# isxml/YOLO-SOMI

Measured on AMD Instinct MI355X. Metric: images/sec train (forward+loss+backward+Adam+EMA) @640, VisDrone-shaped synthetic, yolov5l-SOMI (DCNv3 blocks), higher is better.
Workload: dtype f32; 1 GPU; yolov5l-SOMI (DCNv3 blocks) training step: uint8 ingest + forward (batch-stat BN) + ComputeLoss + backward + Adam + EMA, 640x640, batch 32/GPU (BASELINE configs[1] shape); batch_per_gpu=32, imgsz=640, params=77918970, classes=10, parallelism=dp1

## Files before the change

### yolo-somi_amd/csrc/common.h

```cpp
#pragma once
#include <hip/hip_runtime.h>
#include <stdint.h>
#include <stdio.h>
#include <initializer_list>
#include "../../include/somi_hip.h"

namespace somi {

void set_error(const char *fmt, ...);

#define SOMI_REQUIRE(cond, code, ...)            \
    do {                                         \
        if (!(cond)) {                           \
            ::somi::set_error(__VA_ARGS__);      \
            return (code);                       \
        }                                        \
    } while (0)

static inline int launch_status(const char *what) {
    hipError_t e = hipGetLastError();
    if (e != hipSuccess) {
        set_error("%s: launch failed: %s", what, hipGetErrorString(e));
        return (int)e;
    }
    return 0;
}

static inline bool aligned16(const void *p) { return (reinterpret_cast<uintptr_t>(p) & 15u) == 0; }
static inline int cdiv(long a, long b) { return (int)((a + b - 1) / b); }
static inline int r4(int c) { return (c + 3) / 4 * 4; }
static inline size_t align_up(size_t v, size_t a) { return (v + a - 1) / a * a; }

static inline const char *slice_fault(const void *p, int cs, int coff, int width) {
    if (!p) return "null pointer";
    if (!aligned16(p)) return "base not 16-byte aligned";
    if (cs <= 0 || cs % 4) return "channel stride not a positive multiple of 4";
    if (coff < 0 || coff % 4) return "channel offset not a non-negative multiple of 4";
    if (width <= 0) return "no channels";
    if ((long)coff + width > cs) return "runs past the channel stride";
    return nullptr;
}

struct Slice { const char *name; const void *p; int cs, coff, width; bool optional; };
constexpr bool kOptional = true;
static inline int slices_status(const char *who, std::initializer_list<Slice> slices) {
    for (const Slice &s : slices)
        if (const char *why = s.optional && !s.p ? nullptr : slice_fault(s.p, s.cs, s.coff, s.width)) {
            set_error("%s: %s = [%d, %ld) of %d channels: %s", who, s.name, s.coff, (long)s.coff + s.width, s.cs, why);
            return SOMI_EINVAL;
        }
    return 0;
}
#define SOMI_REQUIRE_SLICES(who, ...)                                          \
    do {                                                                       \
        if (::somi::slices_status(who, {__VA_ARGS__})) return SOMI_EINVAL;     \
    } while (0)

constexpr int kNumXCD = 8;

void launch_dwconv3x3(bool flip, const float *x, const float *w, const float *bias, const float *ps, const float *pt, const float *res,
                      float *y, int B, int H, int W, int C, int act, hipStream_t s);

__device__ __forceinline__ int xcd_remap(int bid, int nblk) {
    const int q = nblk / kNumXCD, r = nblk % kNumXCD;
    const int xcd = bid % kNumXCD, idx = bid / kNumXCD;
    const int start = xcd < r ? xcd * (q + 1) : r * (q + 1) + (xcd - r) * q;
    return start + idx;
}

__device__ __forceinline__ float sigmoidf_(float v) { return 1.0f / (1.0f + expf(-v)); }

__device__ __forceinline__ void bifpn_norm(const float *__restrict__ w, int n_in, float eps, float (&wn)[3]) {
    float s = 0.f;
    for (int i = 0; i < n_in; ++i) s += w[i] * (1.0f / (1.0f + expf(-w[i])));
    for (int i = 0; i < 3; ++i) wn[i] = i < n_in ? w[i] / (s + eps) : 0.f;
}

template <int ACT>
__device__ __forceinline__ float apply_act(float v) {
    if constexpr (ACT == SOMI_ACT_SILU) return v / (1.0f + expf(-v));
    else if constexpr (ACT == SOMI_ACT_GELU) return 0.5f * v * (1.0f + erff(v * 0.70710678118654752440f));
    else if constexpr (ACT == SOMI_ACT_RELU) return fmaxf(v, 0.0f);
    else if constexpr (ACT == SOMI_ACT_SIGMOID) return 1.0f / (1.0f + expf(-v));
    else if constexpr (ACT == SOMI_ACT_LEAKY) return v > 0.0f ? v : 0.1f * v;
    else return v;
}

__device__ __forceinline__ float apply_act_rt(float v, int act) {
    switch (act) {
        case SOMI_ACT_SILU: return apply_act<SOMI_ACT_SILU>(v);
        case SOMI_ACT_GELU: return apply_act<SOMI_ACT_GELU>(v);
        case SOMI_ACT_RELU: return apply_act<SOMI_ACT_RELU>(v);
        case SOMI_ACT_SIGMOID: return apply_act<SOMI_ACT_SIGMOID>(v);
        case SOMI_ACT_LEAKY: return apply_act<SOMI_ACT_LEAKY>(v);
        default: return v;
    }
}

}
```

### yolo-somi_amd/csrc/conv_igemm.hip

```cpp
#include "common.h"

namespace somi {

typedef float f32x16 __attribute__((ext_vector_type(16)));
typedef float f32x4 __attribute__((ext_vector_type(4)));
typedef unsigned u32x4 __attribute__((ext_vector_type(4)));
typedef unsigned u32x2 __attribute__((ext_vector_type(2)));
typedef __bf16 bf16x8 __attribute__((ext_vector_type(8)));

constexpr int BK = 32;
constexpr int OP_LD = BK;
constexpr unsigned OOB = 0xFFFFFFE0u;
constexpr unsigned OOB_BASE = 0xF0000000u;
constexpr unsigned MAX_BUF_BYTES = 0xE0000000u;

__device__ __forceinline__ void lds_dma16(__amdgpu_buffer_rsrc_t r, float *lds_base, unsigned voff) {
#if defined(__HIP_DEVICE_COMPILE__)
    __builtin_amdgcn_raw_ptr_buffer_load_lds(r, (__attribute__((address_space(3))) void *)lds_base, 16, voff, 0, 0, 0);
#endif
}
__device__ __forceinline__ void lds_dma_wait() {
#if defined(__HIP_DEVICE_COMPILE__)
    asm volatile("s_waitcnt vmcnt(0)" ::: "memory");
#endif
// ... 201 lines not shown
        for (int i = 0; i < A_ROWS; ++i) a_par[i] = 0;
#pragma unroll
        for (int i = 0; i < A_ROWS; ++i) {
            const int m = m0 + row0 + RPP * i;
            if (m < Mrows) {
                const int b = m / HoWo + bz, rem = m % HoWo;
                const int ho = h0 + (rem / Wc) * cstep, wo = w0 + (rem % Wc) * cstep;
                if (!a.dgrad) {
                    a_hi0[i] = ho * d.stride - d.pad;
                    a_wi0[i] = wo * d.stride - d.pad;
                } else {
                    a_hi0[i] = (ho + d.pad) / d.stride;
                    a_wi0[i] = (wo + d.pad) / d.stride;
                    a_par[i] = ((ho + d.pad) % d.stride) | (((wo + d.pad) % d.stride) << 8);
                }
                a_pixi[i] = (b * d.H + a_hi0[i]) * d.W + a_wi0[i];
                a_off[i] = a_pixi[i] * d.x_cs + d.x_coff;
                a_chn[i] = b * d.Cin;
            } else {
                a_hi0[i] = -(1 << 28);
                a_wi0[i] = 0; a_pixi[i] = 0; a_off[i] = 0; a_chn[i] = 0;
            }
        }
        unsigned b_off[B_ROWS];
#pragma unroll
        for (int i = 0; i < B_ROWS; ++i) {
            const int n = n0 + row0 + RPP * i;
            b_off[i] = n < d.Cout ? (unsigned)(((size_t)bz * d.Cout + n) * a.K + kc) * 4u : (FAST ? OOB_BASE : OOB);
        }
        unsigned a_mask[A_ROWS], a_offb[A_ROWS], a_pixb[A_ROWS], a_chnb[A_ROWS];
        if constexpr (FAST) {
            const int ntap = nr_c * nq_c;
#pragma unroll
            for (int i = 0; i < A_ROWS; ++i) {
                unsigned mk = 0;
                for (int t = 0; t < ntap; ++t) {
                    const int tr = t / nq_c, tq = t % nq_c;
                    const int hh = a_hi0[i] + (cls ? -tr : tr * d.dil);
                    const int ww = a_wi0[i] + (cls ? -tq : tq * d.dil);
                    mk |= ((unsigned)hh < (unsigned)d.H && (unsigned)ww < (unsigned)d.W) ? (1u << t) : 0u;
                }
                a_mask[i] = mk;
                a_offb[i] = (unsigned)(a_off[i] + kc) * 4u;
                a_pixb[i] = (unsigned)a_pixi[i] * 4u;
                a_chnb[i] = (unsigned)(a_chn[i] + kc) * 4u;
            }
        }
        const int ntap_u = FAST ? nr_c * nq_c : 1;
        int tp_u = FAST ? kt0 % ntap_u : 0, c0_u = FAST ? (kt0 / ntap_u) * BK : 0;
        int r_u = tp_u / nq_c, q_u = tp_u % nq_c;

        int k = kc, c = kc % d.Cin, tap = kc / d.Cin;
        int r = tap / d.kw, q = tap % d.kw;

        f32x4 ra[A_ROWS], rb[B_ROWS];
        auto fetch_tile = [&](int kt_next) {
            if constexpr (FAST) {
                const int dpix = cls ? -(r_u * d.W + q_u) : (r_u * d.W + q_u) * d.dil;
                const unsigned sd = (unsigned)(dpix * d.x_cs + c0_u) * 4u, bit = 1u << tp_u;
#pragma unroll
                for (int i = 0; i < A_ROWS; ++i) {
                    const bool ok = (a_mask[i] & bit) != 0;
                    f32x4 v = buf_load4(rx, ok ? a_offb[i] + sd : OOB);
                    if constexpr (MODULATE) {
                        if (has_chan) v *= buf_load4(rc, ok ? a_chnb[i] + (unsigned)c0_u * 4u : OOB);
                        if (has_pix) v *= buf_load1(rp, ok ? a_pixb[i] + (unsigned)dpix * 4u : OOB);
                    }
                    ra[i] = v;
                }
                const unsigned ko = cls ? (unsigned)(((ph + cstep * r_u) * d.kw + pw + cstep * q_u) * d.Cin + c0_u) * 4u
                                        : (unsigned)(tp_u * d.Cin + c0_u) * 4u;
#pragma unroll
                for (int i = 0; i < B_ROWS; ++i) rb[i] = buf_load4(rw, b_off[i] + ko);
                return;
            }
            const bool kin = k < a.K;
            const int dh = a.dgrad ? -(r / d.stride) : r * d.dil, dw = a.dgrad ? -(q / d.stride) : q * d.dil;
            const int dpix = dh * d.W + dw;
            const int delta = dpix * d.x_cs + c;
            const int rpar = a.dgrad ? ((r % d.stride) | ((q % d.stride) << 8)) : 0;
#pragma unroll
            for (int i = 0; i < A_ROWS; ++i) {
                const bool ok = kin && a_par[i] == rpar && (unsigned)(a_hi0[i] + dh) < (unsigned)d.H &&
                                (unsigned)(a_wi0[i] + dw) < (unsigned)d.W;
                f32x4 v = buf_load4(rx, ok ? (unsigned)(a_off[i] + delta) * 4u : OOB);
                if constexpr (MODULATE) {
                    if (has_chan) v *= buf_load4(rc, ok ? (unsigned)(a_chn[i] + c) * 4u : OOB);
                    if (has_pix) v *= buf_load1(rp, ok ? (unsigned)(a_pixi[i] + dpix) * 4u : OOB);
                }
                ra[i] = v;
            }
#pragma unroll
            for (int i = 0; i < B_ROWS; ++i) rb[i] = buf_load4(rw, (kin && b_off[i] != OOB) ? b_off[i] : OOB);
        };
        auto advance_k = [&]() {
            if constexpr (FAST) {
                ++tp_u;
                if (++q_u == nq_c) { q_u = 0; ++r_u; }
                if (tp_u == ntap_u) {
                    tp_u = 0; r_u = 0; q_u = 0;
                    c0_u += BK;
                }
                return;
            }
            k += BK;
            c += BK;
            while (c >= d.Cin) {
                c -= d.Cin;
                if (++q == d.kw) { q = 0; ++r; }
            }
#pragma unroll
            for (int i = 0; i < B_ROWS; ++i) b_off[i] += (b_off[i] != OOB) ? BK * 4u : 0u;
        };
        auto store_split = [&](float *rowp, const f32x4 &v) {
            const __bf16 h0 = (__bf16)v[0], h1 = (__bf16)v[1], h2 = (__bf16)v[2], h3 = (__bf16)v[3];
            typedef __bf16 bf16x4 __attribute__((ext_vector_type(4)));
            *reinterpret_cast<bf16x4 *>(rowp + st_off) = bf16x4{h0, h1, h2, h3};
            if constexpr (NS == 2) {
                const bf16x4 lo = {(__bf16)(v[0] - (float)h0), (__bf16)(v[1] - (float)h1), (__bf16)(v[2] - (float)h2), (__bf16)(v[3] - (float)h3)};
                *reinterpret_cast<bf16x4 *>(rowp + (st_off ^ 16)) = lo;
            }
        };
        auto store_tile = [&](float *buf) {
            if constexpr (NS != 0) {
#pragma unroll
                for (int i = 0; i < A_ROWS; ++i) store_split(&buf[(row0 + RPP * i) * OP_LD], ra[i]);
#pragma unroll
                for (int i = 0; i < B_ROWS; ++i) store_split(&buf[(BM + row0 + RPP * i) * OP_LD], rb[i]);
                return;
            }
#pragma unroll
            for (int i = 0; i < A_ROWS; ++i)
                *reinterpret_cast<f32x4 *>(&buf[(row0 + RPP * i) * OP_LD + lds_col]) = ra[i];
#pragma unroll
            for (int i = 0; i < B_ROWS; ++i)
                *reinterpret_cast<f32x4 *>(&buf[(BM + row0 + RPP * i) * OP_LD + lds_col]) = rb[i];
        };
        auto dma_tile = [&](float *buf) {
            if constexpr (DMA) {
                const int dpix = cls ? -(r_u * d.W + q_u) : (r_u * d.W + q_u) * d.dil;
                const unsigned sd = (unsigned)(dpix * d.x_cs + c0_u) * 4u, bit = 1u << tp_u;
                float *wrow = buf + wave * 8 * OP_LD;
#pragma unroll
                for (int i = 0; i < A_ROWS; ++i)
                    lds_dma16(rx, wrow + RPP * i * OP_LD, (a_mask[i] & bit) ? a_offb[i] + sd : OOB);
                const unsigned ko = cls ? (unsigned)(((ph + cstep * r_u) * d.kw + pw + cstep * q_u) * d.Cin + c0_u) * 4u
                                        : (unsigned)(tp_u * d.Cin + c0_u) * 4u;
#pragma unroll
                for (int i = 0; i < B_ROWS; ++i)
                    lds_dma16(rw, wrow + (BM + RPP * i) * OP_LD, b_off[i] + ko);
            }
        };

        f32x16 acc[TN][TM];
#pragma unroll
        for (int jn = 0; jn < TN; ++jn)
#pragma unroll
            for (int i = 0; i < TM; ++i)
#pragma unroll
                for (int e = 0; e < 16; ++e) acc[jn][i][e] = 0.f;

        auto load_frag = [&](const float *buf, int j, f32x4 (&fa)[TM], f32x4 (&fb)[TN]) {
#pragma unroll
            for (int i = 0; i < TM; ++i) fa[i] = *reinterpret_cast<const f32x4 *>(buf + aw_off + i * 32 * OP_LD + fo[j]);
#pragma unroll
            for (int i = 0; i < TN; ++i) fb[i] = *reinterpret_cast<const f32x4 *>(buf + bw_off + i * 32 * OP_LD + fo[j]);
        };
        auto mma_steps = [&](const f32x4 (&fa)[TM], const f32x4 (&fb)[TN], int t_lo, int t_hi) {
#pragma unroll
            for (int t = t_lo; t < t_hi; ++t)
#pragma unroll
                for (int jn = 0; jn < TN; ++jn)
#pragma unroll
                    for (int i = 0; i < TM; ++i)
                        acc[jn][i] = __builtin_amdgcn_mfma_f32_32x32x2f32(fb[jn][t], fa[i][t], acc[jn][i], 0, 0, 0);
        };

        if (kt1 > kt0) {
            if constexpr (DMA) {
                dma_tile(lds);
                lds_dma_wait();
            } else {
                fetch_tile(kt0);
                store_tile(lds);
            }
        }
        __syncthreads();
        if constexpr (NS != 0) {
            for (int kt = kt0; kt < kt1; ++kt) {
                const float *cur = lds + ((kt - kt0) & 1) * TILE;
                float *nxt = lds + ((kt - kt0 + 1) & 1) * TILE;
                const bool more = kt + 1 < kt1;
#pragma unroll
                for (int st = 0; st < 2; ++st) {
                    bf16x8 ah[TM], bh[TN], al[TM], bl[TN];
#pragma unroll
                    for (int i = 0; i < TM; ++i) {
                        const float *p = cur + aw_off + i * 32 * OP_LD;
                        ah[i] = *reinterpret_cast<const bf16x8 *>(p + fo16[st]);
                        if constexpr (NS == 2) al[i] = *reinterpret_cast<const bf16x8 *>(p + (fo16[st] ^ 16));
                    }
#pragma unroll
                    for (int i = 0; i < TN; ++i) {
                        const float *p = cur + bw_off + i * 32 * OP_LD;
                        bh[i] = *reinterpret_cast<const bf16x8 *>(p + fo16[st]);
                        if constexpr (NS == 2) bl[i] = *reinterpret_cast<const bf16x8 *>(p + (fo16[st] ^ 16));
                    }
                    if (st == 0 && more) {
                        advance_k();
                        fetch_tile(kt + 1);
                    }
#pragma unroll
                    for (int jn = 0; jn < TN; ++jn)
#pragma unroll
                        for (int i = 0; i < TM; ++i) {
                            if constexpr (NS == 2) {
                                acc[jn][i] = __builtin_amdgcn_mfma_f32_32x32x16_bf16(bl[jn], ah[i], acc[jn][i], 0, 0, 0);
                                acc[jn][i] = __builtin_amdgcn_mfma_f32_32x32x16_bf16(bh[jn], al[i], acc[jn][i], 0, 0, 0);
                            }
                            acc[jn][i] = __builtin_amdgcn_mfma_f32_32x32x16_bf16(bh[jn], ah[i], acc[jn][i], 0, 0, 0);
                        }
                }
                if (more) store_tile(nxt);
                __syncthreads();
            }
        }
        f32x4 fa0[TM], fb0[TN], fa1[TM], fb1[TN];
        if (NS == 0 && kt1 > kt0) load_frag(lds, 0, fa0, fb0);
        for (int kt = kt0; NS == 0 && kt < kt1; ++kt) {
            const float *cur = lds + ((kt - kt0) & 1) * TILE;
            float *nxt = lds + ((kt - kt0 + 1) & 1) * TILE;
            const bool more = kt + 1 < kt1;
            load_frag(cur, 1, fa1, fb1);
            __builtin_amdgcn_sched_barrier(0);
            mma_steps(fa0, fb0, 0, 4);
            if (more) {
                advance_k();
                if constexpr (DMA) dma_tile(nxt);
                else fetch_tile(kt + 1);
            }
            __builtin_amdgcn_sched_barrier(0);
            load_frag(cur, 2, fa0, fb0);
            __builtin_amdgcn_sched_barrier(0);
            mma_steps(fa1, fb1, 0, 4);
            __builtin_amdgcn_sched_barrier(0);
            load_frag(cur, 3, fa1, fb1);
            __builtin_amdgcn_sched_barrier(0);
            mma_steps(fa0, fb0, 0, 4);
            if constexpr (!DMA) {
                if (more) store_tile(nxt);
            }
            __builtin_amdgcn_sched_barrier(0);
            mma_steps(fa1, fb1, 0, 1);
            if constexpr (DMA) lds_dma_wait();
            __syncthreads();
            if (more) load_frag(nxt, 0, fa0, fb0);
            __builtin_amdgcn_sched_barrier(0);
            mma_steps(fa1, fb1, 1, 4);
        }

        if (!sk || (kt0 == 0 && kt1 == nkt)) {
            conv_epilogue<BM, BN, WAVES_M, WAVES_N>(acc, lds, a, rmap, m0, n0);
        } else {
            const bool first_piece = (long)tile * nkt + kt0 == u_lo;
            float *slot = a.ws + ((size_t)wg * 2 + (first_piece ? 0 : 1)) * (BM * BN);
#pragma unroll
            for (int jn = 0; jn < TN; ++jn)
#pragma unroll
                for (int i = 0; i < TM; ++i)
#pragma unroll
                    for (int e = 0; e < 16; ++e) slot[((jn * TM + i) * 16 + e) * NT + tid] = acc[jn][i][e];
        }
        __syncthreads();
    }
}

template <int BM, int BN, int WAVES_M, int WAVES_N>
__global__ __launch_bounds__(WAVES_M * WAVES_N * 64, WAVES_M * WAVES_N / 2) void conv_streamk_fixup_kernel(const ConvArgs a, int G) {
    constexpr int WM = BM / WAVES_M, WN = BN / WAVES_N, TM = WM / 32, TN = WN / 32, NT = WAVES_M * WAVES_N * 64;
    __shared__ __attribute__((aligned(16))) float lds[TileLds<BM, BN, WAVES_M, WAVES_N>::FLOATS];
    const int nkt = a.K / BK, ntile = a.tiles_m * a.tiles_n;
    const long U = (long)ntile * nkt;
    const int g = blockIdx.x + 1;
    const long b = sk_lo(g, U, G);
    if (b % nkt == 0) return;
    const int tile = (int)(b / nkt);
    const long t_lo = (long)tile * nkt, t_hi = t_lo + nkt;
    if (sk_lo(g - 1, U, G) > t_lo) return;
    const int tid = threadIdx.x;
    f32x16 acc[TN][TM];
#pragma unroll
    for (int jn = 0; jn < TN; ++jn)
#pragma unroll
        for (int i = 0; i < TM; ++i)
#pragma unroll
            for (int e = 0; e < 16; ++e) acc[jn][i][e] = 0.f;
    auto slot_of = [&](int w) -> const float * {
        const long lo = sk_lo(w, U, G), hi = sk_lo(w + 1, U, G);
        if (w >= G || lo >= t_hi) return nullptr;
        if (hi <= t_lo || hi == lo) return a.ws;
        const long seg = lo > t_lo ? lo : t_lo;
        return a.ws + ((size_t)w * 2 + (seg == lo ? 0 : 1)) * (BM * BN);
    };
    auto live = [&](int w) {
        const long lo = sk_lo(w, U, G), hi = sk_lo(w + 1, U, G);
        return w < G && lo < t_hi && hi > t_lo && hi != lo;
    };
    for (int w = g - 1; w < G; w += 2) {
        const float *s0 = slot_of(w), *s1 = slot_of(w + 1);
        if (!s0) break;
        const bool l0 = live(w), l1 = s1 && live(w + 1);
        f32x16 t0[TN][TM], t1[TN][TM];
#pragma unroll
        for (int jn = 0; jn < TN; ++jn)
#pragma unroll
            for (int i = 0; i < TM; ++i)
#pragma unroll
                for (int e = 0; e < 16; ++e) {
                    const int o = ((jn * TM + i) * 16 + e) * NT + tid;
                    t0[jn][i][e] = l0 ? s0[o] : 0.f;
                    t1[jn][i][e] = l1 ? s1[o] : 0.f;
                }
#pragma unroll
        for (int jn = 0; jn < TN; ++jn)
#pragma unroll
            for (int i = 0; i < TM; ++i)
#pragma unroll
                for (int e = 0; e < 16; ++e) {
                    if (l0) acc[jn][i][e] += t0[jn][i][e];
                    if (l1) acc[jn][i][e] += t1[jn][i][e];
                }
        if (!s1) break;
    }
    const RowMap rmap = {a.M, a.d.Ho * a.d.Wo, a.d.Wo, 1, 0, 0, 0, false};
    conv_epilogue<BM, BN, WAVES_M, WAVES_N>(acc, lds, a, rmap, (tile / a.tiles_n) * BM, (tile % a.tiles_n) * BN);
}

struct TilePlan {
    int variant;
    bool sk;
};
static const int kTileBM[4] = {128, 64, 128, 128}, kTileBN[4] = {128, 128, 64, 32};

static bool fast_path(const somi_conv_desc &d) {
    return d.Cin % BK == 0 && d.kh * d.kw <= 32 && (size_t)d.kh * d.kw * d.Cin * 4 < (1u << 27);
}
static inline int sk_slots(int variant, const somi_conv_desc &d) {
    const bool three = variant == 2 && !d.a_chan_scale && !d.a_pix_scale && d.prec != 1 && d.prec != 2 && fast_path(d);
    return three ? SK_GRID * 3 / 2 : SK_GRID;
}

static TilePlan plan_tiles(const somi_conv_desc &d, int M, int dgrad) {
    const bool sk_ok = d.workspace && fast_path(d) && !d.per_sample_w && !(dgrad && d.stride > 1);
    TilePlan p{0, false};
    const long blocks128 = (long)cdiv(M, 128) * cdiv(d.Cout, 128) * (d.per_sample_w ? d.B : 1);
    if (d.Cout > 64) {
        if (cdiv(d.Cout, 64) * 64 * 5 <= cdiv(d.Cout, 128) * 128 * 4 && M >= 128 * 256) p.variant = 2;
        else p.variant = (sk_ok || blocks128 >= 512 || M >= 128 * 256) ? 0 : 1;
    } else {
        p.variant = d.Cout > 32 ? 2 : 3;
    }
    if (sk_ok) {
        const int bm = kTileBM[p.variant], bn = kTileBN[p.variant];
        const long ntile = (long)cdiv(M, bm) * cdiv(d.Cout, bn), nkt = (long)d.kh * d.kw * d.Cin / BK;
        const int slots = sk_slots(p.variant, d);
        const long rounds = (ntile + slots - 1) / slots;
        p.sk = ntile * 100 < rounds * slots * 90 && ntile * nkt >= 32 &&
               d.workspace_bytes >= (size_t)slots * 2 * bm * bn * sizeof(float);
    }
    return p;
}

template <int BM, int BN, int WAVES_M, int WAVES_N>
static int launch(const ConvArgs &a, const TilePlan &tp, hipStream_t s) {
    ConvArgs args = a;
    const bool sk = tp.sk;
    const bool mod = a.d.a_chan_scale || a.d.a_pix_scale;
    const bool fast = fast_path(a.d);
    args.cls = a.dgrad && fast;
    args.sk = sk ? 1 : 0;
    args.ws = static_cast<float *>(a.d.workspace);
    const int st = a.d.stride, ncls = args.cls ? st * st : 1;
    const int m_cls = args.cls ? (a.d.per_sample_w ? 1 : a.d.B) * cdiv(a.d.Ho, st) * cdiv(a.d.Wo, st) : a.M;
    args.tiles_m = cdiv(m_cls, BM);
    args.tiles_n = cdiv(a.d.Cout, BN);
    int sk_grid = sk_slots(tp.variant, a.d);
    if (sk) {
        const long U = (long)args.tiles_m * args.tiles_n * (a.K / BK);
        if (U / 8 < sk_grid) sk_grid = (int)(U / 8);
        if (sk_grid < 2) sk_grid = 2;
    }
    const dim3 grid(sk ? sk_grid : args.tiles_m * args.tiles_n, ncls, a.d.per_sample_w ? a.d.B : 1);
    auto fixup = [&] {
        if (sk) hipLaunchKernelGGL((conv_streamk_fixup_kernel<BM, BN, WAVES_M, WAVES_N>), dim3(sk_grid - 1), dim3(WAVES_M * WAVES_N * 64), 0, s, args, sk_grid);
    };
    if constexpr (WAVES_M * WAVES_N == 8) {
        if (a.ns && fast && !mod) {
            if (a.ns == 1)
                hipLaunchKernelGGL((conv_igemm_f32_kernel<BM, BN, WAVES_M, WAVES_N, false, true, 1>), grid, dim3(WAVES_M * WAVES_N * 64), 0, s, args);
            else
                hipLaunchKernelGGL((conv_igemm_f32_kernel<BM, BN, WAVES_M, WAVES_N, false, true, 2>), grid, dim3(WAVES_M * WAVES_N * 64), 0, s, args);
            fixup();
            return launch_status("somi_conv2d_nhwc_f32 (bf16)");
        }
    }
    if (mod && fast)
        hipLaunchKernelGGL((conv_igemm_f32_kernel<BM, BN, WAVES_M, WAVES_N, true, true>), grid, dim3(WAVES_M * WAVES_N * 64), 0, s, args);
    else if (mod)
        hipLaunchKernelGGL((conv_igemm_f32_kernel<BM, BN, WAVES_M, WAVES_N, true, false>), grid, dim3(WAVES_M * WAVES_N * 64), 0, s, args);
    else if (fast)
        hipLaunchKernelGGL((conv_igemm_f32_kernel<BM, BN, WAVES_M, WAVES_N, false, true>), grid, dim3(WAVES_M * WAVES_N * 64), 0, s, args);
    else
        hipLaunchKernelGGL((conv_igemm_f32_kernel<BM, BN, WAVES_M, WAVES_N, false, false>), grid, dim3(WAVES_M * WAVES_N * 64), 0, s, args);
    fixup();
    return launch_status("somi_conv2d_nhwc_f32");
}

}

namespace somi {
static int conv_launch(const somi_conv_desc *dp, somi_stream_t stream, int dgrad) {
    SOMI_REQUIRE(dp, SOMI_EINVAL, "conv: null descriptor");
    const somi_conv_desc &d = *dp;
    SOMI_REQUIRE(d.w && aligned16(d.w), SOMI_EINVAL, "conv: the weights must be given and 16 B aligned");
    SOMI_REQUIRE(d.B > 0 && d.H > 0 && d.W > 0 && d.Cin > 0 && d.Cout > 0, SOMI_EINVAL, "conv: empty shape");
// ... 114 lines not shown
```

### yolo-somi_amd/csrc/conv_wgrad.hip

```cpp
#include "common.h"

namespace somi {

typedef float f32x16 __attribute__((ext_vector_type(16)));
typedef float f32x4 __attribute__((ext_vector_type(4)));
typedef unsigned u32x4 __attribute__((ext_vector_type(4)));
typedef __bf16 bf16x8 __attribute__((ext_vector_type(8)));
typedef __bf16 bf16x4 __attribute__((ext_vector_type(4)));
typedef short i16x4 __attribute__((ext_vector_type(4)));
typedef short i16x8 __attribute__((ext_vector_type(8)));

constexpr int WG_PIX = 32;
constexpr unsigned W_OOB = 0xFFFFFFE0u;
constexpr unsigned W_MAX_BUF = 0xE0000000u;

struct WgradArgs {
    const float *x, *dy;
    float *out;
    int B, H, W, Cin, x_cs, x_coff, Ho, Wo, Cout, dy_cs, dy_coff, kh, kw, stride, pad;
    int K;
    int tiles_co, tiles_k, splits, pix_per_split, npix;
    int bm, bn;
    int per_sample;
    unsigned x_bytes, dy_bytes;
    int ns;
};

__device__ __forceinline__ f32x4 wbuf_load4(__amdgpu_buffer_rsrc_t r, unsigned off) {
    return __builtin_bit_cast(f32x4, __builtin_amdgcn_raw_buffer_load_b128(r, off, 0, 0));
}

__device__ __forceinline__ void lds_dma16(__amdgpu_buffer_rsrc_t r, float *lds_base, unsigned voff) {
#if defined(__HIP_DEVICE_COMPILE__)
    __builtin_amdgcn_raw_ptr_buffer_load_lds(r, (__attribute__((address_space(3))) void *)lds_base, 16, voff, 0, 0, 0);
#endif
}
__device__ __forceinline__ void lds_dma_wait() {
#if defined(__HIP_DEVICE_COMPILE__)
    asm volatile("s_waitcnt vmcnt(0)" ::: "memory");
#endif
}

__device__ __forceinline__ i16x4 lds_read_tr16(const char *p) {
#if defined(__HIP_DEVICE_COMPILE__)
    return __builtin_amdgcn_ds_read_tr16_b64_v4i16((__attribute__((address_space(3))) i16x4 *)p);
#else
    return i16x4{0, 0, 0, 0};
#endif
}

template <int BM, int BN, int NW = 4, int NS = 0>
__global__ __launch_bounds__(NW * 64, NW / 2) void conv_wgrad_f32_kernel(const WgradArgs a) {
    constexpr int NT = NW * 64;
    static_assert(NS == 0 || ((BM == 128 || BM == 64) && BN == 128 && NW == 8), "the bf16 forms exist for the 128 / 64 x 128 tiles with 8 waves");
    constexpr int WAVES_N = NW == 8 ? 4 : (BM == 64 ? 2 : 1), WAVES_M = NW / WAVES_N;
    static_assert(BM / WAVES_M >= 32 && BN / WAVES_N >= 32, "bad wgrad tiling");
    constexpr int WM = BM / WAVES_M, WN = BN / WAVES_N, TM = WM / 32, TN = WN / 32;
    constexpr int A_LD = BM, B_LD = BN;
    constexpr int TILE = WG_PIX * (A_LD + B_LD);
    constexpr int BUF = NS ? 8192 : TILE;
    __shared__ __attribute__((aligned(16))) float lds[2 * BUF];

    const int tid = threadIdx.x, lane = tid & 63;
    const int wave = __builtin_amdgcn_readfirstlane(tid >> 6);
    const int wm = wave / WAVES_N, wn = wave % WAVES_N;
    const int ntile = a.tiles_co * a.tiles_k;
    const int lid = xcd_remap(blockIdx.x, ntile * a.splits);
    const int tile = lid % ntile, split = lid / ntile, set = blockIdx.z;
    const int tile_k = tile % a.tiles_k, tile_co = tile / a.tiles_k;
    const int co0 = tile_co * BM, k0 = tile_k * BN;

    const __amdgpu_buffer_rsrc_t rx = __builtin_amdgcn_make_buffer_rsrc((void *)a.x, 0, a.x_bytes, 0x00020000);
    const __amdgpu_buffer_rsrc_t rdy = __builtin_amdgcn_make_buffer_rsrc((void *)a.dy, 0, a.dy_bytes, 0x00020000);

    const int p_lo = split * a.pix_per_split, p_hi = min(p_lo + a.pix_per_split, a.npix);
    const long set_pix0 = (long)set * a.npix;

    constexpr int A_QUADS = BM / 4, B_QUADS = BN / 4;
    constexpr int A_ROWS_PER_PASS = NT / A_QUADS, B_ROWS_PER_PASS = NT / B_QUADS;
    const int a_quad = tid % A_QUADS, a_row0 = tid / A_QUADS;
    const int b_quad = tid % B_QUADS, b_row0 = tid / B_QUADS;
    const int b_col = k0 + b_quad * 4;
    const bool a_col_ok = co0 + a_quad * 4 < a.Cout, b_col_ok = b_col < a.K;
    const int b_tap = b_col / a.Cin, b_ci = b_col % a.Cin;
    const int r = b_tap / a.kw, q = b_tap % a.kw;
    constexpr int A_N = WG_PIX / A_ROWS_PER_PASS, B_N = WG_PIX / B_ROWS_PER_PASS;

    int bb[B_N], bho[B_N], bwo[B_N];
    const int HoWo = a.Ho * a.Wo;
#pragma unroll
    for (int i = 0; i < B_N; ++i) {
        const long P = set_pix0 + p_lo + b_row0 + i * B_ROWS_PER_PASS;
        bb[i] = (int)(P / HoWo);
        const int rem = (int)(P % HoWo);
        bho[i] = rem / a.Wo;
        bwo[i] = rem % a.Wo;
    }
    const unsigned set_p0 = (unsigned)(set_pix0 + p_lo);
    const unsigned a_col = (unsigned)(a.dy_coff + co0 + a_quad * 4), b_colo = (unsigned)(a.x_coff + b_ci);
    const int npl = p_hi - p_lo;
    auto advance = [&]() {
#pragma unroll
        for (int i = 0; i < B_N; ++i) {
            bwo[i] += WG_PIX;
            while (bwo[i] >= a.Wo) {
                bwo[i] -= a.Wo;
                if (++bho[i] == a.Ho) { bho[i] = 0; ++bb[i]; }
            }
        }
    };
    auto dma = [&](float *buf, int pt) {
        float *wbase = buf + wave * 256;
#pragma unroll
        for (int i = 0; i < A_N; ++i) {
            const int pl = pt + a_row0 + i * A_ROWS_PER_PASS;
            const bool ok = a_col_ok && pl < npl;
            const unsigned off = ((set_p0 + (unsigned)pl) * (unsigned)a.dy_cs + a_col) * 4u;
            lds_dma16(rdy, wbase + i * A_ROWS_PER_PASS * A_LD, ok ? off : W_OOB);
        }
#pragma unroll
        for (int i = 0; i < B_N; ++i) {
            const int pl = pt + b_row0 + i * B_ROWS_PER_PASS;
            const int hi = bho[i] * a.stride - a.pad + r, wi = bwo[i] * a.stride - a.pad + q;
            const bool ok = b_col_ok && pl < npl && (unsigned)hi < (unsigned)a.H && (unsigned)wi < (unsigned)a.W;
            const unsigned off = ((unsigned)((bb[i] * a.H + hi) * a.W + wi) * (unsigned)a.x_cs + b_colo) * 4u;
            lds_dma16(rx, wbase + WG_PIX * A_LD + i * B_ROWS_PER_PASS * B_LD, ok ? off : W_OOB);
        }
    };

    f32x4 ra[A_N], rb[B_N];
    auto fetch = [&](int pt) {
#pragma unroll
        for (int i = 0; i < A_N; ++i) {
            const int pl = pt + a_row0 + i * A_ROWS_PER_PASS;
            const bool ok = a_col_ok && pl < npl;
            const unsigned off = ((set_p0 + (unsigned)pl) * (unsigned)a.dy_cs + a_col) * 4u;
            ra[i] = wbuf_load4(rdy, ok ? off : W_OOB);
        }
#pragma unroll
        for (int i = 0; i < B_N; ++i) {
            const int pl = pt + b_row0 + i * B_ROWS_PER_PASS;
            const int hi = bho[i] * a.stride - a.pad + r, wi = bwo[i] * a.stride - a.pad + q;
            const bool ok = b_col_ok && pl < npl && (unsigned)hi < (unsigned)a.H && (unsigned)wi < (unsigned)a.W;
            const unsigned off = ((unsigned)((bb[i] * a.H + hi) * a.W + wi) * (unsigned)a.x_cs + b_colo) * 4u;
            rb[i] = wbuf_load4(rx, ok ? off : W_OOB);
        }
    };
    auto split_store = [&](char *img, int row, int quad, const f32x4 &v) {
        const int key = ((row & 3) << 2) | ((row >> 2) & 3);
        char *p = img + 256 * row + 16 * ((quad >> 1) ^ key) + 8 * (quad & 1);
        const __bf16 h0 = (__bf16)v[0], h1 = (__bf16)v[1], h2 = (__bf16)v[2], h3 = (__bf16)v[3];
        *reinterpret_cast<bf16x4 *>(p) = bf16x4{h0, h1, h2, h3};
        if constexpr (NS == 2)
            *reinterpret_cast<bf16x4 *>(p + 8192) = bf16x4{(__bf16)(v[0] - (float)h0), (__bf16)(v[1] - (float)h1), (__bf16)(v[2] - (float)h2),
                                                           (__bf16)(v[3] - (float)h3)};
    };
    auto store_bf16 = [&](float *buf) {
        char *img = reinterpret_cast<char *>(buf);
#pragma unroll
        for (int i = 0; i < A_N; ++i) split_store(img, a_row0 + i * A_ROWS_PER_PASS, a_quad, ra[i]);
#pragma unroll
        for (int i = 0; i < B_N; ++i) split_store(img + 16384, b_row0 + i * B_ROWS_PER_PASS, b_quad, rb[i]);
    };

    f32x16 acc[TM][TN];
#pragma unroll
    for (int i = 0; i < TM; ++i)
#pragma unroll
        for (int j = 0; j < TN; ++j)
#pragma unroll
            for (int e = 0; e < 16; ++e) acc[i][j][e] = 0.f;

    const int nkt = (p_hi - p_lo + WG_PIX - 1) / WG_PIX;
    const int a_frag = (lane >> 5) * A_LD + wm * WM + (lane & 31);
    const int b_frag = WG_PIX * A_LD + (lane >> 5) * B_LD + wn * WN + (lane & 31);
    auto mma_quarter = [&](const float *buf, int qtr) {
#pragma unroll
        for (int ks = qtr * 4; ks < qtr * 4 + 4; ++ks) {
            float fa[TM], fb[TN];
#pragma unroll
            for (int i = 0; i < TM; ++i) fa[i] = buf[a_frag + ks * 2 * A_LD + i * 32];
#pragma unroll
            for (int j = 0; j < TN; ++j) fb[j] = buf[b_frag + ks * 2 * B_LD + j * 32];
#pragma unroll
            for (int i = 0; i < TM; ++i)
#pragma unroll
                for (int j = 0; j < TN; ++j) acc[i][j] = __builtin_amdgcn_mfma_f32_32x32x2f32(fa[i], fb[j], acc[i][j], 0, 0, 0);
        }
    };

    if constexpr (NS != 0) {
        const int h = lane >> 5, cg = (lane >> 4) & 1, q4 = (lane & 15) >> 2, p4 = lane & 3;
        int lpart[2];
#pragma unroll
        for (int jj = 0; jj < 2; ++jj) {
            const int keylo = (2 * h + jj) & 3;
            lpart[jj] = 256 * (8 * h + 4 * jj + q4) + 16 * ((2 * cg + (p4 >> 1)) ^ keylo) + 8 * (p4 & 1);
        }
        int ta[TM], tb[TN];
#pragma unroll
        for (int i = 0; i < TM; ++i) ta[i] = 16 * ((((wm * WM + i * 32) >> 3)) ^ (q4 << 2));
#pragma unroll
        for (int j = 0; j < TN; ++j) tb[j] = 16384 + 16 * ((((wn * WN + j * 32) >> 3)) ^ (q4 << 2));
        auto frag = [&](const char *img, int off) -> bf16x8 {
            const i16x4 lo4 = lds_read_tr16(img + off + lpart[0]), hi4 = lds_read_tr16(img + off + lpart[1]);
            return __builtin_bit_cast(bf16x8, i16x8{lo4[0], lo4[1], lo4[2], lo4[3], hi4[0], hi4[1], hi4[2], hi4[3]});
        };
        if (nkt > 0) {
            fetch(0);
            store_bf16(lds);
        }
        __syncthreads();
        for (int kt = 0; kt < nkt; ++kt) {
            const char *cur = reinterpret_cast<const char *>(lds + (kt & 1) * BUF);
            float *nxt = lds + ((kt + 1) & 1) * BUF;
            const bool more = kt + 1 < nkt;
#pragma unroll
            for (int st = 0; st < 2; ++st) {
                bf16x8 ah[TM], al[TM], bh[TN], bl[TN];
#pragma unroll
                for (int i = 0; i < TM; ++i) {
                    ah[i] = frag(cur, 4096 * st + ta[i]);
                    if constexpr (NS == 2) al[i] = frag(cur, 8192 + 4096 * st + ta[i]);
                }
#pragma unroll
                for (int j = 0; j < TN; ++j) {
                    bh[j] = frag(cur, 4096 * st + tb[j]);
                    if constexpr (NS == 2) bl[j] = frag(cur, 8192 + 4096 * st + tb[j]);
                }
                if (st == 0 && more) {
                    advance();
                    fetch((kt + 1) * WG_PIX);
                }
#pragma unroll
                for (int i = 0; i < TM; ++i)
#pragma unroll
                    for (int j = 0; j < TN; ++j) {
                        if constexpr (NS == 2) {
                            acc[i][j] = __builtin_amdgcn_mfma_f32_32x32x16_bf16(al[i], bh[j], acc[i][j], 0, 0, 0);
                            acc[i][j] = __builtin_amdgcn_mfma_f32_32x32x16_bf16(ah[i], bl[j], acc[i][j], 0, 0, 0);
                        }
                        acc[i][j] = __builtin_amdgcn_mfma_f32_32x32x16_bf16(ah[i], bh[j], acc[i][j], 0, 0, 0);
                    }
            }
            if (more) store_bf16(nxt);
            __syncthreads();
        }
    }
    if (NS == 0 && nkt > 0) {
        dma(lds, 0);
        lds_dma_wait();
    }
    __syncthreads();
    for (int kt = 0; NS == 0 && kt < nkt; ++kt) {
        const float *cur = lds + (kt & 1) * TILE;
        float *nxt = lds + ((kt + 1) & 1) * TILE;
        const bool more = kt + 1 < nkt;
        mma_quarter(cur, 0);
        if (more) {
            advance();
            dma(nxt, (kt + 1) * WG_PIX);
        }
        mma_quarter(cur, 1);
        mma_quarter(cur, 2);
        mma_quarter(cur, 3);
        lds_dma_wait();
        __syncthreads();
    }

    float *out = a.out + ((size_t)split * gridDim.z + set) * a.Cout * a.K;
#pragma unroll
    for (int j = 0; j < TN; ++j) {
        const int kcol = k0 + wn * WN + j * 32 + (lane & 31);
        if (kcol >= a.K) continue;
#pragma unroll
        for (int i = 0; i < TM; ++i) {
#pragma unroll
            for (int e = 0; e < 16; ++e) {
                const int co = co0 + wm * WM + i * 32 + (e & 3) + 8 * (e >> 2) + 4 * (lane >> 5);
                if (co < a.Cout) out[(size_t)co * a.K + kcol] = acc[i][j][e];
            }
        }
    }
}

__global__ __launch_bounds__(256) void wgrad_reduce_kernel(const float *__restrict__ part, int splits, long n, const float *accumulate,
                                                           float *__restrict__ dw) {
    __shared__ f32x4 sm[16][16];
    const long n4 = n >> 2;
    const int col = threadIdx.x & 15, grp = threadIdx.x >> 4;
    const f32x4 zero = {0.f, 0.f, 0.f, 0.f};
    for (long i0 = blockIdx.x * 16L; i0 < n4; i0 += (long)gridDim.x * 16) {
        const long i = i0 + col;
        f32x4 s0 = zero, s1 = zero;
        if (i < n4) {
            for (int k = grp; k < splits; k += 64) {
                f32x4 v[4];
#pragma unroll
                for (int u = 0; u < 4; ++u)
                    v[u] = k + u * 16 < splits ? *reinterpret_cast<const f32x4 *>(part + (size_t)(k + u * 16) * n + i * 4) : zero;
                s0 += v[0];
                s1 += v[1];
                s0 += v[2];
                s1 += v[3];
            }
        }
        sm[grp][col] = s0 + s1;
        __syncthreads();
        if (grp == 0 && i < n4) {
            f32x4 s = accumulate ? *reinterpret_cast<const f32x4 *>(accumulate + i * 4) : zero;
#pragma unroll
            for (int g = 0; g < 16; ++g) s += sm[g][col];
            *reinterpret_cast<f32x4 *>(dw + i * 4) = s;
        }
        __syncthreads();
    }
}

static int plan(const somi_conv_desc &f, WgradArgs &a) {
    SOMI_REQUIRE(f.B > 0 && f.H > 0 && f.W > 0 && f.Cin > 0 && f.Cout > 0 && f.kh > 0 && f.kw > 0 && f.stride > 0 && f.pad >= 0,
                 SOMI_EINVAL, "conv wgrad: bad geometry");
    SOMI_REQUIRE(f.dil == 1, SOMI_ENOTIMPL, "conv wgrad: dilation 1 only");
    SOMI_REQUIRE(f.Ho == (f.H + 2 * f.pad - f.kh) / f.stride + 1 && f.Wo == (f.W + 2 * f.pad - f.kw) / f.stride + 1, SOMI_EINVAL,
                 "conv wgrad: Ho/Wo do not match the forward geometry");
    SOMI_REQUIRE(f.Cin % 4 == 0 && f.Cout % 4 == 0, SOMI_EINVAL, "conv wgrad: Cin and Cout must be multiples of 4");
    a.B = f.B; a.H = f.H; a.W = f.W; a.Cin = f.Cin; a.Ho = f.Ho; a.Wo = f.Wo; a.Cout = f.Cout;
    a.kh = f.kh; a.kw = f.kw; a.stride = f.stride; a.pad = f.pad;
    a.K = f.kh * f.kw * f.Cin;
    a.per_sample = f.per_sample_w ? 1 : 0;
    a.npix = a.per_sample ? f.Ho * f.Wo : f.B * f.Ho * f.Wo;
    a.bm = (cdiv(f.Cout, 64) * 64 < cdiv(f.Cout, 128) * 128) ? 64 : 128;
    a.bn = a.K > 64 ? 128 : (a.K > 32 || a.bm == 64 ? 64 : 32);
    a.tiles_co = cdiv(f.Cout, a.bm);
    a.tiles_k = cdiv(a.K, a.bn);
    const long tiles = (long)a.tiles_co * a.tiles_k * (a.per_sample ? f.B : 1);
    long want = 1024 / tiles;
    const long max_splits = (a.npix + WG_PIX * 8 - 1) / (WG_PIX * 8);
    if (want > max_splits) want = max_splits;
    if (want < 1) want = 1;
    a.pix_per_split = (int)(((a.npix + want - 1) / want + WG_PIX - 1) / WG_PIX * WG_PIX);
    a.splits = cdiv(a.npix, a.pix_per_split);
    return 0;
}

}

using namespace somi;

extern "C" size_t somi_conv2d_wgrad_workspace_bytes(const somi_conv_desc *fwd) {
    WgradArgs a{};
    if (!fwd || plan(*fwd, a)) return 0;
    return (size_t)(a.splits < 1 ? 1 : a.splits) * (a.per_sample ? a.B : 1) * a.Cout * a.K * 4 + 256;
}

extern "C" const char *somi_conv2d_wgrad_kernel_name(const somi_conv_desc *fwd) {
    WgradArgs a{};
    if (!fwd || plan(*fwd, a)) return nullptr;
    static thread_local char name[64];
    snprintf(name, sizeof(name), "conv_wgrad_f32_kernel<%d,%d,%d>", a.bm, a.bn, a.bn == 128 ? 8 : 4);
    return name;
}

extern "C" int somi_conv2d_wgrad_nhwc_f32(const somi_conv_desc *fwd, const float *x, int x_cs, int x_coff, const float *dy, int dy_cs,
                                          int dy_coff, float *dw, const float *accumulate, void *workspace, size_t workspace_bytes,
                                          somi_stream_t stream) {
    SOMI_REQUIRE(fwd && dw && aligned16(dw) && workspace, SOMI_EINVAL, "conv wgrad: needs the descriptor, a 16 B aligned dw and the workspace");
    WgradArgs a{};
    int rc = plan(*fwd, a);
    if (rc) return rc;
    SOMI_REQUIRE_SLICES("conv wgrad", {"x", x, x_cs, x_coff, a.Cin}, {"dy", dy, dy_cs, dy_coff, a.Cout});
    SOMI_REQUIRE(workspace_bytes >= somi_conv2d_wgrad_workspace_bytes(fwd), SOMI_EWORKSPACE, "conv wgrad: workspace too small");
    const size_t xb = (size_t)a.B * a.H * a.W * x_cs * 4, yb = (size_t)a.B * a.Ho * a.Wo * dy_cs * 4;
    if (xb > W_MAX_BUF || yb > W_MAX_BUF) {
        SOMI_REQUIRE(!a.per_sample, SOMI_ENOTIMPL, "conv wgrad: per-sample gradients of tensors beyond the 4 GiB descriptor range");
        const size_t per_img = (xb > yb ? xb : yb) / a.B;
        SOMI_REQUIRE(per_img <= W_MAX_BUF, SOMI_ENOTIMPL, "conv wgrad: one image exceeds the 4 GiB descriptor range");
        const int bsub = (int)(W_MAX_BUF / per_img);
        for (int b0 = 0; b0 < a.B; b0 += bsub) {
            somi_conv_desc sub = *fwd;
            sub.B = a.B - b0 < bsub ? a.B - b0 : bsub;
            rc = somi_conv2d_wgrad_nhwc_f32(&sub, x + (size_t)b0 * a.H * a.W * x_cs, x_cs, x_coff, dy + (size_t)b0 * a.Ho * a.Wo * dy_cs, dy_cs,
                                            dy_coff, dw, b0 == 0 ? accumulate : dw, workspace, workspace_bytes, stream);
            if (rc) return rc;
        }
        return 0;
    }
    a.x = x; a.dy = dy; a.x_cs = x_cs; a.x_coff = x_coff; a.dy_cs = dy_cs; a.dy_coff = dy_coff;
    a.x_bytes = (unsigned)xb; a.dy_bytes = (unsigned)yb;
    const int sets = a.per_sample ? a.B : 1;
    const bool direct = a.splits == 1 && !accumulate;
    a.out = direct ? dw : static_cast<float *>(workspace);
    hipStream_t s = static_cast<hipStream_t>(stream);
    const dim3 grid(a.tiles_co * a.tiles_k * a.splits, 1, sets);
    a.ns = (fwd->prec == 1 || fwd->prec == 2) && !a.per_sample && a.bn == 128 ? fwd->prec : 0;
    if (a.ns == 1 && a.bm == 128) hipLaunchKernelGGL((conv_wgrad_f32_kernel<128, 128, 8, 1>), grid, dim3(512), 0, s, a);
    else if (a.ns == 2 && a.bm == 128) hipLaunchKernelGGL((conv_wgrad_f32_kernel<128, 128, 8, 2>), grid, dim3(512), 0, s, a);
    else if (a.ns == 1) hipLaunchKernelGGL((conv_wgrad_f32_kernel<64, 128, 8, 1>), grid, dim3(512), 0, s, a);
    else if (a.ns == 2) hipLaunchKernelGGL((conv_wgrad_f32_kernel<64, 128, 8, 2>), grid, dim3(512), 0, s, a);
    else if (a.bm == 128 && a.bn == 128) hipLaunchKernelGGL((conv_wgrad_f32_kernel<128, 128, 8>), grid, dim3(512), 0, s, a);
    else if (a.bm == 128 && a.bn == 64) hipLaunchKernelGGL((conv_wgrad_f32_kernel<128, 64>), grid, dim3(256), 0, s, a);
    else if (a.bm == 128) hipLaunchKernelGGL((conv_wgrad_f32_kernel<128, 32>), grid, dim3(256), 0, s, a);
    else if (a.bn == 128) hipLaunchKernelGGL((conv_wgrad_f32_kernel<64, 128, 8>), grid, dim3(512), 0, s, a);
    else hipLaunchKernelGGL((conv_wgrad_f32_kernel<64, 64>), grid, dim3(256), 0, s, a);
    if (!direct) {
        const long n = (long)sets * a.Cout * a.K;
        long g = (n / 4 + 15) / 16;
        hipLaunchKernelGGL(wgrad_reduce_kernel, dim3((unsigned)(g > 4096 ? 4096 : (g < 1 ? 1 : g))), dim3(256), 0, s,
                           static_cast<const float *>(workspace), a.splits, n, accumulate, dw);
    }
    return launch_status("somi_conv2d_wgrad_nhwc_f32");
}
```

Before: 99.22 images/s.

## Add late-wave software-pipelined schedule for 8-wave fp32 conv wgrad kernel

Adds a LATE variant of the 8-wave fp32 weight-gradient kernel. In it, the upper four waves preload LDS fragments for a quarter into registers and issue the MFMAs for earlier quarters, carrying two quarters across k-tile iterations, so LDS reads overlap matrix math. It is enabled by default when each split covers at least 8 k-tiles, and an environment variable can override the choice. The cost is many more registers per thread in those waves, which could reduce occupancy or cause spills. The forward igemm change only wraps the body in an inlined lambda.

```diff
diff --git a/yolo-somi_amd/csrc/common.h b/yolo-somi_amd/csrc/common.h
--- a/yolo-somi_amd/csrc/common.h
+++ b/yolo-somi_amd/csrc/common.h
@@ -2,6 +2,7 @@
 #include <hip/hip_runtime.h>
 #include <stdint.h>
 #include <stdio.h>
+#include <stdlib.h>
 #include <initializer_list>
 #include "../../include/somi_hip.h"
 
@@ -58,6 +59,13 @@
 
 constexpr int kNumXCD = 8;
 
+constexpr int kConvSchedLate = 1;
+static inline int conv_sched_mask(int dflt, long kt_per_piece, long late_min_kt) {
+    const char *e = getenv("SOMI_CONV_SCHED");
+    if (e && *e) return atoi(e) & kConvSchedLate;
+    return kt_per_piece >= late_min_kt ? dflt : dflt & ~kConvSchedLate;
+}
+
 void launch_dwconv3x3(bool flip, const float *x, const float *w, const float *bias, const float *ps, const float *pt, const float *res,
                       float *y, int B, int H, int W, int C, int act, hipStream_t s);
 
diff --git a/yolo-somi_amd/csrc/conv_igemm.hip b/yolo-somi_amd/csrc/conv_igemm.hip
--- a/yolo-somi_amd/csrc/conv_igemm.hip
+++ b/yolo-somi_amd/csrc/conv_igemm.hip
@@ -377,6 +377,7 @@
             }
         };
 
+        auto piece = [&]() __attribute__((always_inline)) {
         f32x16 acc[TN][TM];
 #pragma unroll
         for (int jn = 0; jn < TN; ++jn)
@@ -496,6 +497,8 @@
 #pragma unroll
                     for (int e = 0; e < 16; ++e) slot[((jn * TM + i) * 16 + e) * NT + tid] = acc[jn][i][e];
         }
+        };
+        piece();
         __syncthreads();
     }
 }
diff --git a/yolo-somi_amd/csrc/conv_wgrad.hip b/yolo-somi_amd/csrc/conv_wgrad.hip
--- a/yolo-somi_amd/csrc/conv_wgrad.hip
+++ b/yolo-somi_amd/csrc/conv_wgrad.hip
@@ -13,6 +13,7 @@
 constexpr int WG_PIX = 32;
 constexpr unsigned W_OOB = 0xFFFFFFE0u;
 constexpr unsigned W_MAX_BUF = 0xE0000000u;
+constexpr long kWgradLateMinKt = 8;
 
 struct WgradArgs {
     const float *x, *dy;
@@ -49,9 +50,10 @@
 #endif
 }
 
-template <int BM, int BN, int NW = 4, int NS = 0>
+template <int BM, int BN, int NW = 4, int NS = 0, bool LATE = false>
 __global__ __launch_bounds__(NW * 64, NW / 2) void conv_wgrad_f32_kernel(const WgradArgs a) {
     constexpr int NT = NW * 64;
+    static_assert(!LATE || (NW == 8 && NS == 0), "the late half exists for the 8-wave fp32 form only");
     static_assert(NS == 0 || ((BM == 128 || BM == 64) && BN == 128 && NW == 8), "the bf16 forms exist for the 128 / 64 x 128 tiles with 8 waves");
     constexpr int WAVES_N = NW == 8 ? 4 : (BM == 64 ? 2 : 1), WAVES_M = NW / WAVES_N;
     static_assert(BM / WAVES_M >= 32 && BN / WAVES_N >= 32, "bad wgrad tiling");
@@ -252,7 +254,61 @@
         lds_dma_wait();
     }
     __syncthreads();
-    for (int kt = 0; NS == 0 && kt < nkt; ++kt) {
+    const bool late = LATE && wave >= 4;
+    if constexpr (LATE) {
+        if (late) {
+            float a0[4][TM], b0[4][TN], a1[4][TM], b1[4][TN], a2[4][TM], b2[4][TN], a3[4][TM], b3[4][TN];
+            auto load_quarter = [&](const float *buf, int qtr, float (&fa)[4][TM], float (&fb)[4][TN]) {
+#pragma unroll
+                for (int s4 = 0; s4 < 4; ++s4) {
+                    const int ks = qtr * 4 + s4;
+#pragma unroll
+                    for (int i = 0; i < TM; ++i) fa[s4][i] = buf[a_frag + ks * 2 * A_LD + i * 32];
+#pragma unroll
+                    for (int j = 0; j < TN; ++j) fb[s4][j] = buf[b_frag + ks * 2 * B_LD + j * 32];
+                }
+            };
+            auto mma_regs = [&](const float (&fa)[4][TM], const float (&fb)[4][TN]) {
+#pragma unroll
+                for (int s4 = 0; s4 < 4; ++s4)
+#pragma unroll
+                    for (int i = 0; i < TM; ++i)
+#pragma unroll
+                        for (int j = 0; j < TN; ++j) acc[i][j] = __builtin_amdgcn_mfma_f32_32x32x2f32(fa[s4][i], fb[s4][j], acc[i][j], 0, 0, 0);
+            };
+            for (int kt = 0; kt < nkt; ++kt) {
+                const float *cur = lds + (kt & 1) * TILE;
+                float *nxt = lds + ((kt + 1) & 1) * TILE;
+                const bool more = kt + 1 < nkt, carried = kt > 0;
+                load_quarter(cur, 0, a0, b0);
+                __builtin_amdgcn_sched_barrier(0);
+                if (carried) mma_regs(a2, b2);
+                if (more) {
+                    advance();
+                    dma(nxt, (kt + 1) * WG_PIX);
+                }
+                __builtin_amdgcn_sched_barrier(0);
+                load_quarter(cur, 1, a1, b1);
+                __builtin_amdgcn_sched_barrier(0);
+                if (carried) mma_regs(a3, b3);
+                __builtin_amdgcn_sched_barrier(0);
+                load_quarter(cur, 2, a2, b2);
+                __builtin_amdgcn_sched_barrier(0);
+                mma_regs(a0, b0);
+                __builtin_amdgcn_sched_barrier(0);
+                load_quarter(cur, 3, a3, b3);
+                __builtin_amdgcn_sched_barrier(0);
+                mma_regs(a1, b1);
+                lds_dma_wait();
+                __syncthreads();
+            }
+            if (nkt > 0) {
+                mma_regs(a2, b2);
+                mma_regs(a3, b3);
+            }
+        }
+    }
+    for (int kt = 0; NS == 0 && !late && kt < nkt; ++kt) {
         const float *cur = lds + (kt & 1) * TILE;
         float *nxt = lds + ((kt + 1) & 1) * TILE;
         const bool more = kt + 1 < nkt;
@@ -393,10 +449,13 @@
     hipStream_t s = static_cast<hipStream_t>(stream);
     const dim3 grid(a.tiles_co * a.tiles_k * a.splits, 1, sets);
     a.ns = (fwd->prec == 1 || fwd->prec == 2) && !a.per_sample && a.bn == 128 ? fwd->prec : 0;
+    const bool late = a.ns == 0 && a.bn == 128 && (conv_sched_mask(kConvSchedLate, a.pix_per_split / WG_PIX, kWgradLateMinKt) & kConvSchedLate);
     if (a.ns == 1 && a.bm == 128) hipLaunchKernelGGL((conv_wgrad_f32_kernel<128, 128, 8, 1>), grid, dim3(512), 0, s, a);
     else if (a.ns == 2 && a.bm == 128) hipLaunchKernelGGL((conv_wgrad_f32_kernel<128, 128, 8, 2>), grid, dim3(512), 0, s, a);
     else if (a.ns == 1) hipLaunchKernelGGL((conv_wgrad_f32_kernel<64, 128, 8, 1>), grid, dim3(512), 0, s, a);
     else if (a.ns == 2) hipLaunchKernelGGL((conv_wgrad_f32_kernel<64, 128, 8, 2>), grid, dim3(512), 0, s, a);
+    else if (a.bm == 128 && a.bn == 128 && late) hipLaunchKernelGGL((conv_wgrad_f32_kernel<128, 128, 8, 0, true>), grid, dim3(512), 0, s, a);
+    else if (a.bn == 128 && late) hipLaunchKernelGGL((conv_wgrad_f32_kernel<64, 128, 8, 0, true>), grid, dim3(512), 0, s, a);
     else if (a.bm == 128 && a.bn == 128) hipLaunchKernelGGL((conv_wgrad_f32_kernel<128, 128, 8>), grid, dim3(512), 0, s, a);
     else if (a.bm == 128 && a.bn == 64) hipLaunchKernelGGL((conv_wgrad_f32_kernel<128, 64>), grid, dim3(256), 0, s, a);
     else if (a.bm == 128) hipLaunchKernelGGL((conv_wgrad_f32_kernel<128, 32>), grid, dim3(256), 0, s, a);
```

Result: no change. 99.71 images/s (median of 6 runs) (+0.5%).
